# HaSai666/rec_pangu

Hardware: AMD Instinct MI355X
Metric: samples/sec DeepFM Criteo-shape bsz=65536/GPU (train step: fwd+bwd+dense Adam+zero_grad) (higher is better)
Workload: dtype f32

## Files before the change

### rec_pangu_amd/csrc/embed_tiny.hip

```cpp
#include "common.h"
#include "bfsplit.h"

#define ET_MAXF 16
#define ET_ROWS 224
#define ET_COLS 160
#define ET_LD 72
#define ET_CHUNK 64
#define ET_NOROW 254
#define ET_NOSMP 255

struct TinyTables {
    int n, total;
    int field[ET_MAXF];
    int base[ET_MAXF];
    int rows[ET_MAXF];
    int acc0[ET_MAXF];
};

__device__ __forceinline__ void tiny_split3(float v, __bf16 *p0, __bf16 *p1, __bf16 *p2) {
    uint32_t u = __float_as_uint(v);
    *reinterpret_cast<uint16_t *>(p0) = (uint16_t)(u >> 16);
    v -= __uint_as_float(u & 0xFFFF0000u);
    u = __float_as_uint(v);
    *reinterpret_cast<uint16_t *>(p1) = (uint16_t)(u >> 16);
    v -= __uint_as_float(u & 0xFFFF0000u);
    u = __float_as_uint(v);
    *reinterpret_cast<uint16_t *>(p2) = (uint16_t)(u >> 16);
}

__global__ __launch_bounds__(256, 2) void embed_grad_tiny_partial_kernel(
    const int32_t *__restrict__ keys, int64_t B, TinyTables tt, const float *__restrict__ dh, int64_t lddh,
    const float *__restrict__ sum_in, const float *__restrict__ gfm, int64_t per_blk, float *__restrict__ partial) {
    __shared__ __attribute__((aligned(16))) __bf16 Zt[3][ET_COLS][ET_LD];
    __shared__ __attribute__((aligned(8))) uint8_t rid[ET_MAXF][ET_CHUNK];
    __shared__ uint8_t rfld[ET_ROWS], rloc[ET_ROWS];
    const int t = threadIdx.x, wv = t >> 6, l = t & 63, i = l & 31, h = l >> 5;
    for (int m = t; m < ET_ROWS; m += 256) {
        int slot = 0, loc = ET_NOROW;
        for (int j = 0; j < tt.n; ++j)
            if (m >= tt.acc0[j] && m < tt.acc0[j] + tt.rows[j]) {
                slot = j;
                loc = m - tt.acc0[j];
            }
        rfld[m] = (uint8_t)slot;
        rloc[m] = (uint8_t)loc;
    }
    for (int e = t; e < 3 * (ET_COLS - 130) * ET_LD; e += 256) {
        const int p = e / ((ET_COLS - 130) * ET_LD), rest = e - p * ((ET_COLS - 130) * ET_LD);
        Zt[p][130 + rest / ET_LD][rest % ET_LD] = (__bf16)0.f;
    }
    f32x16 acc[5];
#pragma unroll
    for (int nt = 0; nt < 5; ++nt)
#pragma unroll
        for (int r = 0; r < 16; ++r) acc[nt][r] = 0.f;
    const int64_t s_begin = (int64_t)blockIdx.x * per_blk;
    const int64_t s_end = s_begin + per_blk < B ? s_begin + per_blk : B;
    __syncthreads();
    const int mt = 4 * (int)blockIdx.y + wv;
    const bool mok = mt < ET_ROWS / 32;
    const int fl0 = mok ? rfld[32 * mt + i] : 0, lc0 = mok ? rloc[32 * mt + i] : ET_NOROW;
    const int s = t >> 2, q = t & 3;
    f32x4 vd[4], vs[4];
    float g = 0.f, okf = 0.f;
    int rloc0 = ET_NOSMP, rloc1 = ET_NOSMP;
    auto fetch = [&](int64_t c0) {
        const int64_t b = c0 + s;
        const bool ok = b < s_end;
        const int64_t bc = ok ? b : s_end - 1;
        okf = ok ? 1.f : 0.f;
        g = (gfm != nullptr) ? gfm[bc] * okf : 0.f;
#pragma unroll
        for (int e = 0; e < 4; ++e) vd[e] = *reinterpret_cast<const f32x4 *>(dh + bc * lddh + 16 * q + 4 * e);
        if (sum_in != nullptr) {
#pragma unroll
            for (int e = 0; e < 4; ++e) vs[e] = *reinterpret_cast<const f32x4 *>(sum_in + bc * 64 + 16 * q + 4 * e);
        }
        rloc0 = rloc1 = ET_NOSMP;
        {
            const int idx = t, j = idx >> 6, ss = idx & 63;
            if (idx < tt.n * ET_CHUNK && c0 + ss < s_end) rloc0 = keys[(int64_t)tt.field[j] * B + c0 + ss] - tt.base[j];
        }
        {
            const int idx = t + 256, j = idx >> 6, ss = idx & 63;
            if (idx < tt.n * ET_CHUNK && c0 + ss < s_end) rloc1 = keys[(int64_t)tt.field[j] * B + c0 + ss] - tt.base[j];
        }
    };
    fetch(s_begin);
    for (int64_t c0 = s_begin; c0 < s_end; c0 += ET_CHUNK) {
        {
#pragma unroll
            for (int e = 0; e < 16; ++e) {
                const int col = 16 * q + e;
                tiny_split3(vd[e >> 2][e & 3] * okf, &Zt[0][col][s], &Zt[1][col][s], &Zt[2][col][s]);
                const float uval = (sum_in != nullptr) ? g * vs[e >> 2][e & 3] : 0.f;
                tiny_split3(uval, &Zt[0][64 + col][s], &Zt[1][64 + col][s], &Zt[2][64 + col][s]);
            }
            if (q == 0) tiny_split3(g, &Zt[0][128][s], &Zt[1][128][s], &Zt[2][128][s]);
            if (q == 1) tiny_split3(okf, &Zt[0][129][s], &Zt[1][129][s], &Zt[2][129][s]);
            if (t < tt.n * ET_CHUNK) rid[t >> 6][t & 63] = (uint8_t)rloc0;
            if (t + 256 < tt.n * ET_CHUNK) rid[(t + 256) >> 6][t & 63] = (uint8_t)rloc1;
            for (int idx = t + 512; idx < tt.n * ET_CHUNK; idx += 256) {
                const int j = idx >> 6, ss = idx & 63;
                int loc = ET_NOSMP;
                if (c0 + ss < s_end) loc = keys[(int64_t)tt.field[j] * B + c0 + ss] - tt.base[j];
                rid[j][ss] = (uint8_t)loc;
            }
        }
        if (c0 + ET_CHUNK < s_end) fetch(c0 + ET_CHUNK);
        __syncthreads();
#pragma unroll
        for (int ks = 0; ks < 4; ++ks) {
            const uint64_t r8 = *reinterpret_cast<const uint64_t *>(&rid[fl0][16 * ks + 8 * h]);
            u32x4 aw;
#pragma unroll
            for (int j = 0; j < 4; ++j) {
                const uint32_t e0 = (uint32_t)((r8 >> (16 * j)) & 0xFF), e1 = (uint32_t)((r8 >> (16 * j + 8)) & 0xFF);
                aw[j] = (e0 == (uint32_t)lc0 ? 0x00003F80u : 0u) | (e1 == (uint32_t)lc0 ? 0x3F800000u : 0u);
            }
            const bf16x8 a = __builtin_bit_cast(bf16x8, aw);
            if (mok) {
#pragma unroll
                for (int nt = 0; nt < 5; ++nt)
#pragma unroll
                    for (int p = 2; p >= 0; --p) {
                        const bf16x8 bq = *reinterpret_cast<const bf16x8 *>(&Zt[p][32 * nt + i][16 * ks + 8 * h]);
                        acc[nt] = __builtin_amdgcn_mfma_f32_32x32x16_bf16(a, bq, acc[nt], 0, 0, 0);
                    }
            }
        }
        __syncthreads();
    }
    float *P = partial + (int64_t)blockIdx.x * ET_ROWS * ET_COLS;
    if (mok) {
#pragma unroll
        for (int nt = 0; nt < 5; ++nt)
#pragma unroll
            for (int r = 0; r < 16; ++r)
                P[(int64_t)(32 * mt + (r & 3) + 8 * (r >> 2) + 4 * h) * ET_COLS + 32 * nt + i] = acc[nt][r];
    }
}

#define ET_FIN_PARTS 4
__global__ __launch_bounds__(ET_COLS * ET_FIN_PARTS) void embed_grad_tiny_finish_kernel(
    const float *__restrict__ partial, int nblk, TinyTables tt, const float *__restrict__ wt, int64_t ldwt,
    const float *__restrict__ arena, float *__restrict__ G, int accumulate, int has_fm, float *__restrict__ hs_out) {
    __shared__ float Sp[ET_FIN_PARTS][ET_COLS];
    __shared__ float S[ET_COLS];
    const int m = blockIdx.x, c = threadIdx.x % ET_COLS, part = threadIdx.x / ET_COLS;
    int slot = 0;
    for (int j = 0; j < tt.n; ++j)
        if (m >= tt.acc0[j] && m < tt.acc0[j] + tt.rows[j]) slot = j;
    const int64_t arow = (int64_t)tt.base[slot] + (m - tt.acc0[slot]);
    {
        const int per = (nblk + ET_FIN_PARTS - 1) / ET_FIN_PARTS;
        const int b0 = part * per, b1 = (b0 + per < nblk) ? b0 + per : nblk;
        float s = 0.f;
#pragma unroll 8
        for (int b = b0; b < b1; ++b) s += partial[((int64_t)b * ET_ROWS + m) * ET_COLS + c];
        Sp[part][c] = s;
    }
    __syncthreads();
    if (threadIdx.x < ET_COLS) S[c] = (Sp[0][c] + Sp[1][c]) + (Sp[2][c] + Sp[3][c]);
    __syncthreads();
    if (hs_out != nullptr && threadIdx.x >= 64 && threadIdx.x < 128) hs_out[m * 64 + (threadIdx.x - 64)] = S[threadIdx.x - 64];
    if (threadIdx.x < 64) {
        const int d = threadIdx.x;
        const float *w = wt + ((int64_t)tt.field[slot] * 64 + d) * ldwt;
        float a = 0.f;
#pragma unroll 8
        for (int hh = 0; hh < 64; ++hh) a = __builtin_fmaf(S[hh], w[hh], a);
        a += S[64 + d];
        if (has_fm) a -= S[128] * arena[arow * 64 + d];
        float *dst = G + arow * 64 + d;
        if (S[129] > 0.f) *dst = accumulate ? *dst + a : a;
    }
}

__global__ __launch_bounds__(256) void embed_grad_tiny_dw_kernel(const float *__restrict__ hs, TinyTables tt,
                                                                 const float *__restrict__ arena, float *__restrict__ dw,
                                                                 int64_t lddw) {
    const int slot = (int)blockIdx.x;
    const int e = (int)blockIdx.y * 256 + (int)threadIdx.x, d = e & 63, hh = e >> 6;
    const float *hrow = hs + (int64_t)tt.acc0[slot] * 64 + hh;
    const float *vrow = arena + (int64_t)tt.base[slot] * 64 + d;
    float a = 0.f;
    const int nr = tt.rows[slot];
    int r = 0;
    for (; r + 8 <= nr; r += 8) {
        float hv[8], vv[8];
#pragma unroll
        for (int u = 0; u < 8; ++u) {
            hv[u] = hrow[(int64_t)(r + u) * 64];
            vv[u] = vrow[(int64_t)(r + u) * 64];
        }
#pragma unroll
        for (int u = 0; u < 8; ++u) a = __builtin_fmaf(hv[u], vv[u], a);
    }
    for (; r < nr; ++r) a = __builtin_fmaf(hrow[(int64_t)r * 64], vrow[(int64_t)r * 64], a);
    dw[(int64_t)hh * lddw + (int64_t)tt.field[slot] * 64 + d] = a;
}

static int64_t tiny_per_block(int64_t B) {
    int64_t per = rp_cdiv(rp_cdiv(B, 128), ET_CHUNK) * ET_CHUNK;
    return per < ET_CHUNK ? ET_CHUNK : per;
}

extern "C" int rp_embed_grad_tiny_workspace_bytes(int64_t B, size_t *bytes) {
    RP_REQUIRE(bytes && B >= 1, "embed_grad_tiny_workspace_bytes: bad argument");
    *bytes = (size_t)rp_cdiv(B, tiny_per_block(B)) * ET_ROWS * ET_COLS * sizeof(float) + (size_t)ET_ROWS * 64 * sizeof(float) + 256;
    return RP_OK;
}

extern "C" int rp_embed_grad_tiny(const int32_t *keys, int64_t B, const int32_t *tiny_field, const int64_t *tiny_base,
                                  const int32_t *tiny_rows, int n_tiny, const float *dh, int64_t lddh, const float *wt,
                                  int64_t ldwt, const float *gfm, const float *sum_in, const float *arena,
                                  float *grad_arena, int accumulate, float *dw, int64_t lddw, void *workspace,
                                  size_t workspace_bytes, rp_stream_t stream) {
    RP_REQUIRE(keys && tiny_field && tiny_base && tiny_rows && dh && wt && grad_arena && workspace, "embed_grad_tiny: null pointer");
    RP_REQUIRE(n_tiny >= 1 && n_tiny <= ET_MAXF, "embed_grad_tiny: %d tables (1..%d)", n_tiny, ET_MAXF);
    RP_REQUIRE(B >= 1 && B < INT32_MAX, "embed_grad_tiny: bad B");
    RP_REQUIRE(gfm == nullptr || arena != nullptr, "embed_grad_tiny: the FM term needs the arena");
    RP_REQUIRE(lddh % 4 == 0 && ldwt >= 64 && rp_aligned16(dh) && (sum_in == nullptr || rp_aligned16(sum_in)),
               "embed_grad_tiny: dh / sum_in rows must be 16-byte aligned");
    TinyTables tt;
    tt.n = n_tiny;
    int total = 0;
    for (int j = 0; j < ET_MAXF; ++j) {
        tt.field[j] = tt.base[j] = tt.rows[j] = tt.acc0[j] = 0;
        if (j >= n_tiny) continue;
        RP_REQUIRE(tiny_rows[j] >= 1 && tiny_rows[j] <= ET_NOROW, "embed_grad_tiny: table %d has %d rows (1..%d)", j, tiny_rows[j],
                   ET_NOROW);
        RP_REQUIRE(tiny_base[j] >= 0 && tiny_base[j] < INT32_MAX && tiny_field[j] >= 0, "embed_grad_tiny: bad table %d", j);
        tt.field[j] = tiny_field[j];
        tt.base[j] = (int)tiny_base[j];
        tt.rows[j] = tiny_rows[j];
        tt.acc0[j] = total;
        total += tiny_rows[j];
    }
    RP_REQUIRE(total <= ET_ROWS, "embed_grad_tiny: %d rows together (<= %d)", total, ET_ROWS);
    tt.total = total;
    const int64_t per = tiny_per_block(B);
    const int64_t nblk = rp_cdiv(B, per);
    size_t need = 0;
    rp_embed_grad_tiny_workspace_bytes(B, &need);
    RP_REQUIRE(workspace_bytes >= need, "embed_grad_tiny: workspace %zu < %zu bytes", workspace_bytes, need);
    float *partial = reinterpret_cast<float *>((reinterpret_cast<uintptr_t>(workspace) + 255) & ~(uintptr_t)255);
    hipStream_t s = (hipStream_t)stream;
    hipLaunchKernelGGL(embed_grad_tiny_partial_kernel, dim3((unsigned)nblk, 2), dim3(256), 0, s, keys, B, tt, dh, lddh, sum_in, gfm, per,
                       partial);
    RP_LAUNCH_CHECK("embed_grad_tiny (partial sums)");
    RP_REQUIRE(dw == nullptr || arena != nullptr, "embed_grad_tiny: the weight gradient needs the arena");
    float *hs = dw ? partial + (size_t)nblk * ET_ROWS * ET_COLS : nullptr;
    hipLaunchKernelGGL(embed_grad_tiny_finish_kernel, dim3((unsigned)total), dim3(ET_COLS * ET_FIN_PARTS), 0, s, partial, (int)nblk, tt, wt, ldwt, arena,
                       grad_arena, accumulate, gfm != nullptr ? 1 : 0, hs);
    RP_LAUNCH_CHECK("embed_grad_tiny (finish)");
    if (dw != nullptr) {
        for (int j = 0; j < n_tiny; ++j)
            RP_REQUIRE(lddw >= ((int64_t)tt.field[j] + 1) * 64, "embed_grad_tiny: dw rows shorter than field %d's columns", tt.field[j]);
        hipLaunchKernelGGL(embed_grad_tiny_dw_kernel, dim3((unsigned)n_tiny, 16), dim3(256), 0, s, hs, tt, arena, dw, lddw);
        RP_LAUNCH_CHECK("embed_grad_tiny (weight gradient)");
    }
    return RP_OK;
}
```

Baseline: 89.14 million.

## Double-buffer tiny embedding grad staging and merge row halves into one block

New measurement: 89.24 million, median of 3. No clear change (+0.1%).

```diff
diff --git a/rec_pangu_amd/csrc/embed_tiny.hip b/rec_pangu_amd/csrc/embed_tiny.hip
--- a/rec_pangu_amd/csrc/embed_tiny.hip
+++ b/rec_pangu_amd/csrc/embed_tiny.hip
@@ -17,25 +17,25 @@
     int acc0[ET_MAXF];
 };
 
-__device__ __forceinline__ void tiny_split3(float v, __bf16 *p0, __bf16 *p1, __bf16 *p2) {
-    uint32_t u = __float_as_uint(v);
-    *reinterpret_cast<uint16_t *>(p0) = (uint16_t)(u >> 16);
-    v -= __uint_as_float(u & 0xFFFF0000u);
-    u = __float_as_uint(v);
-    *reinterpret_cast<uint16_t *>(p1) = (uint16_t)(u >> 16);
-    v -= __uint_as_float(u & 0xFFFF0000u);
-    u = __float_as_uint(v);
-    *reinterpret_cast<uint16_t *>(p2) = (uint16_t)(u >> 16);
-}
-
-__global__ __launch_bounds__(256, 2) void embed_grad_tiny_partial_kernel(
+__device__ __forceinline__ void tiny_split3_pair(float a, float b, uint32_t (&w)[3]) {
+#pragma unroll
+    for (int p = 0; p < 3; ++p) {
+        const uint32_t ua = __float_as_uint(a), ub = __float_as_uint(b);
+        w[p] = (ua >> 16) | (ub & 0xFFFF0000u);
+        a -= __uint_as_float(ua & 0xFFFF0000u);
+        b -= __uint_as_float(ub & 0xFFFF0000u);
+    }
+}
+
+#define ET_THREADS 512
+__global__ __launch_bounds__(ET_THREADS) void embed_grad_tiny_partial_kernel(
     const int32_t *__restrict__ keys, int64_t B, TinyTables tt, const float *__restrict__ dh, int64_t lddh,
     const float *__restrict__ sum_in, const float *__restrict__ gfm, int64_t per_blk, float *__restrict__ partial) {
-    __shared__ __attribute__((aligned(16))) __bf16 Zt[3][ET_COLS][ET_LD];
-    __shared__ __attribute__((aligned(8))) uint8_t rid[ET_MAXF][ET_CHUNK];
+    __shared__ __attribute__((aligned(16))) __bf16 Zt[2][3][ET_COLS][ET_LD];
+    __shared__ __attribute__((aligned(8))) uint8_t rid[2][ET_MAXF][ET_CHUNK];
     __shared__ uint8_t rfld[ET_ROWS], rloc[ET_ROWS];
     const int t = threadIdx.x, wv = t >> 6, l = t & 63, i = l & 31, h = l >> 5;
-    for (int m = t; m < ET_ROWS; m += 256) {
+    for (int m = t; m < ET_ROWS; m += ET_THREADS) {
         int slot = 0, loc = ET_NOROW;
         for (int j = 0; j < tt.n; ++j)
             if (m >= tt.acc0[j] && m < tt.acc0[j] + tt.rows[j]) {
@@ -45,9 +45,9 @@
         rfld[m] = (uint8_t)slot;
         rloc[m] = (uint8_t)loc;
     }
-    for (int e = t; e < 3 * (ET_COLS - 130) * ET_LD; e += 256) {
+    for (int e = t; e < 6 * (ET_COLS - 130) * ET_LD; e += ET_THREADS) {
         const int p = e / ((ET_COLS - 130) * ET_LD), rest = e - p * ((ET_COLS - 130) * ET_LD);
-        Zt[p][130 + rest / ET_LD][rest % ET_LD] = (__bf16)0.f;
+        Zt[p / 3][p % 3][130 + rest / ET_LD][rest % ET_LD] = (__bf16)0.f;
     }
     f32x16 acc[5];
 #pragma unroll
@@ -57,61 +57,72 @@
     const int64_t s_begin = (int64_t)blockIdx.x * per_blk;
     const int64_t s_end = s_begin + per_blk < B ? s_begin + per_blk : B;
     __syncthreads();
-    const int mt = 4 * (int)blockIdx.y + wv;
+    const int mt = wv;
     const bool mok = mt < ET_ROWS / 32;
     const int fl0 = mok ? rfld[32 * mt + i] : 0, lc0 = mok ? rloc[32 * mt + i] : ET_NOROW;
-    const int s = t >> 2, q = t & 3;
-    f32x4 vd[4], vs[4];
-    float g = 0.f, okf = 0.f;
-    int rloc0 = ET_NOSMP, rloc1 = ET_NOSMP;
+    const int sp = (l & 7) + 8 * (wv & 3), q = (l >> 3) + 8 * (wv >> 2);
+    f32x4 vd[2], vs[2];
+    float graw[2] = {0.f, 0.f};
+    int kraw0 = 0, kraw1 = 0;
+    const int wvs = __builtin_amdgcn_readfirstlane(wv);
+    const bool has0 = wvs < tt.n, has1 = 8 + wvs < tt.n;
+    const int32_t *key0 = keys + (int64_t)tt.field[wvs] * B, *key1 = keys + (int64_t)tt.field[(8 + wvs) & (ET_MAXF - 1)] * B;
+    const int base0 = tt.base[wvs], base1 = tt.base[(8 + wvs) & (ET_MAXF - 1)];
     auto fetch = [&](int64_t c0) {
-        const int64_t b = c0 + s;
-        const bool ok = b < s_end;
-        const int64_t bc = ok ? b : s_end - 1;
-        okf = ok ? 1.f : 0.f;
-        g = (gfm != nullptr) ? gfm[bc] * okf : 0.f;
-#pragma unroll
-        for (int e = 0; e < 4; ++e) vd[e] = *reinterpret_cast<const f32x4 *>(dh + bc * lddh + 16 * q + 4 * e);
-        if (sum_in != nullptr) {
-#pragma unroll
-            for (int e = 0; e < 4; ++e) vs[e] = *reinterpret_cast<const f32x4 *>(sum_in + bc * 64 + 16 * q + 4 * e);
-        }
-        rloc0 = rloc1 = ET_NOSMP;
-        {
-            const int idx = t, j = idx >> 6, ss = idx & 63;
-            if (idx < tt.n * ET_CHUNK && c0 + ss < s_end) rloc0 = keys[(int64_t)tt.field[j] * B + c0 + ss] - tt.base[j];
-        }
-        {
-            const int idx = t + 256, j = idx >> 6, ss = idx & 63;
-            if (idx < tt.n * ET_CHUNK && c0 + ss < s_end) rloc1 = keys[(int64_t)tt.field[j] * B + c0 + ss] - tt.base[j];
-        }
+#pragma unroll
+        for (int k = 0; k < 2; ++k) {
+            const int64_t b = c0 + 2 * sp + k;
+            const int64_t bc = b < s_end ? b : s_end - 1;
+            if (gfm != nullptr) graw[k] = gfm[bc];
+            vd[k] = *reinterpret_cast<const f32x4 *>(dh + bc * lddh + 4 * q);
+            if (sum_in != nullptr) vs[k] = *reinterpret_cast<const f32x4 *>(sum_in + bc * 64 + 4 * q);
+        }
+        const int64_t bl = c0 + l < s_end ? c0 + l : s_end - 1;
+        if (has0) kraw0 = key0[bl];
+        if (has1) kraw1 = key1[bl];
     };
+    auto stage = [&](int buf, int64_t c0) {
+        float okf[2], g[2];
+#pragma unroll
+        for (int k = 0; k < 2; ++k) {
+            okf[k] = (c0 + 2 * sp + k < s_end) ? 1.f : 0.f;
+            g[k] = (gfm != nullptr) ? graw[k] * okf[k] : 0.f;
+        }
+        uint32_t w[3];
+#pragma unroll
+        for (int e = 0; e < 4; ++e) {
+            const int col = 4 * q + e;
+            tiny_split3_pair(vd[0][e] * okf[0], vd[1][e] * okf[1], w);
+#pragma unroll
+            for (int p = 0; p < 3; ++p) *reinterpret_cast<uint32_t *>(&Zt[buf][p][col][2 * sp]) = w[p];
+            const float u0 = (sum_in != nullptr) ? g[0] * vs[0][e] : 0.f, u1 = (sum_in != nullptr) ? g[1] * vs[1][e] : 0.f;
+            tiny_split3_pair(u0, u1, w);
+#pragma unroll
+            for (int p = 0; p < 3; ++p) *reinterpret_cast<uint32_t *>(&Zt[buf][p][64 + col][2 * sp]) = w[p];
+        }
+        if (q < 2) {
+            tiny_split3_pair(q == 0 ? g[0] : okf[0], q == 0 ? g[1] : okf[1], w);
+#pragma unroll
+            for (int p = 0; p < 3; ++p) *reinterpret_cast<uint32_t *>(&Zt[buf][p][128 + q][2 * sp]) = w[p];
+        }
+        const bool okl = c0 + l < s_end;
+        if (has0) rid[buf][wvs][l] = (uint8_t)(okl ? kraw0 - base0 : ET_NOSMP);
+        if (has1) rid[buf][8 + wvs][l] = (uint8_t)(okl ? kraw1 - base1 : ET_NOSMP);
+    };
+    vs[0] = vs[1] = f32x4{0.f, 0.f, 0.f, 0.f};
+    const int nch = (int)((s_end - s_begin + ET_CHUNK - 1) / ET_CHUNK);
     fetch(s_begin);
-    for (int64_t c0 = s_begin; c0 < s_end; c0 += ET_CHUNK) {
-        {
-#pragma unroll
-            for (int e = 0; e < 16; ++e) {
-                const int col = 16 * q + e;
-                tiny_split3(vd[e >> 2][e & 3] * okf, &Zt[0][col][s], &Zt[1][col][s], &Zt[2][col][s]);
-                const float uval = (sum_in != nullptr) ? g * vs[e >> 2][e & 3] : 0.f;
-                tiny_split3(uval, &Zt[0][64 + col][s], &Zt[1][64 + col][s], &Zt[2][64 + col][s]);
-            }
-            if (q == 0) tiny_split3(g, &Zt[0][128][s], &Zt[1][128][s], &Zt[2][128][s]);
-            if (q == 1) tiny_split3(okf, &Zt[0][129][s], &Zt[1][129][s], &Zt[2][129][s]);
-            if (t < tt.n * ET_CHUNK) rid[t >> 6][t & 63] = (uint8_t)rloc0;
-            if (t + 256 < tt.n * ET_CHUNK) rid[(t + 256) >> 6][t & 63] = (uint8_t)rloc1;
-            for (int idx = t + 512; idx < tt.n * ET_CHUNK; idx += 256) {
-                const int j = idx >> 6, ss = idx & 63;
-                int loc = ET_NOSMP;
-                if (c0 + ss < s_end) loc = keys[(int64_t)tt.field[j] * B + c0 + ss] - tt.base[j];
-                rid[j][ss] = (uint8_t)loc;
-            }
-        }
-        if (c0 + ET_CHUNK < s_end) fetch(c0 + ET_CHUNK);
-        __syncthreads();
+    stage(0, s_begin);
+    fetch(s_begin + ET_CHUNK);
+    __syncthreads();
+    for (int c = 0; c < nch; ++c) {
+        const int buf = c & 1;
+        const int64_t c0 = s_begin + (int64_t)c * ET_CHUNK;
+        if (c + 1 < nch) stage(buf ^ 1, c0 + ET_CHUNK);
+        fetch(c0 + 2 * ET_CHUNK);
 #pragma unroll
         for (int ks = 0; ks < 4; ++ks) {
-            const uint64_t r8 = *reinterpret_cast<const uint64_t *>(&rid[fl0][16 * ks + 8 * h]);
+            const uint64_t r8 = *reinterpret_cast<const uint64_t *>(&rid[buf][fl0][16 * ks + 8 * h]);
             u32x4 aw;
 #pragma unroll
             for (int j = 0; j < 4; ++j) {
@@ -124,7 +135,7 @@
                 for (int nt = 0; nt < 5; ++nt)
 #pragma unroll
                     for (int p = 2; p >= 0; --p) {
-                        const bf16x8 bq = *reinterpret_cast<const bf16x8 *>(&Zt[p][32 * nt + i][16 * ks + 8 * h]);
+                        const bf16x8 bq = *reinterpret_cast<const bf16x8 *>(&Zt[buf][p][32 * nt + i][16 * ks + 8 * h]);
                         acc[nt] = __builtin_amdgcn_mfma_f32_32x32x16_bf16(a, bq, acc[nt], 0, 0, 0);
                     }
             }
@@ -247,7 +258,7 @@
     RP_REQUIRE(workspace_bytes >= need, "embed_grad_tiny: workspace %zu < %zu bytes", workspace_bytes, need);
     float *partial = reinterpret_cast<float *>((reinterpret_cast<uintptr_t>(workspace) + 255) & ~(uintptr_t)255);
     hipStream_t s = (hipStream_t)stream;
-    hipLaunchKernelGGL(embed_grad_tiny_partial_kernel, dim3((unsigned)nblk, 2), dim3(256), 0, s, keys, B, tt, dh, lddh, sum_in, gfm, per,
+    hipLaunchKernelGGL(embed_grad_tiny_partial_kernel, dim3((unsigned)nblk), dim3(ET_THREADS), 0, s, keys, B, tt, dh, lddh, sum_in, gfm, per,
                        partial);
     RP_LAUNCH_CHECK("embed_grad_tiny (partial sums)");
     RP_REQUIRE(dw == nullptr || arena != nullptr, "embed_grad_tiny: the weight gradient needs the arena");
```
